# Mariachiar/Spatiotemporal-Deepfake-Detection-for-Live-Video-Calls

Hardware: AMD Instinct MI355X
Metric: clips/sec (32x3x224x224) (higher is better)
Workload: dtype bf16

## Files before the change

spatiotemporal-deepfake-detection-for-live-video-calls_amd/csrc/af_conv.hip:

```cpp
#include "af_common.h"

namespace af {

struct ConvArgs {
    const char* in;
    const char* w;
    const float* scale;
    const float* shift;
    const char* res;
    char* out;
    int T, H, W, Cin, Cout;
    int CinP, CoutP;
    int kt, kh, kw, st, sh, sw, pt, ph, pw;
    int To, Ho, Wo;
    int relu, out_ld;
    int ring;
    int tpool;
    long long M;
    int tiles_n;
    int kpt;
    const char* in2;
    const char* w2;
    int T2, H2, W2, Cin2, Cin2P, st2, sh2, sw2, kpt2;
    int ksplit;
    unsigned div_w_m, div_w_l, div_h_m, div_h_l, div_t_m, div_t_l;
    float* ws;
    long long ws_bytes;
#ifdef AF_STAMPS
    unsigned long long* stamps;
    int dbg;
#endif
};

template <int DT, int BN, int BM, int WN, int WM, int KS, int NSTAGE, int MINW, bool DUAL, bool SPLITK, int BMR>
__device__ __forceinline__ void conv_igemm_tile(const ConvArgs& a, const int bid, const int nb) {
    typedef Elem<DT> E;
    constexpr int EPC = E::EPC;
    constexpr int ES = 16 / EPC;
    constexpr int WTN = BN / WN, WTM = BMR / WM;
    constexpr int TN = WTN / 16, TM = WTM / 16;
    constexpr int NW = WN * WM * KS;
    constexpr int GR = NW * 8;
    constexpr int RW = BN / GR, RX = BM / GR;
    constexpr int PER_WAVE = RW + RX;
    constexpr int STAGE_BYTES = (BN + BM) * 128;
    static_assert(NW == 8 && (KS == 1 || KS == 2) && BN % GR == 0 && BM % GR == 0, "8 waves per workgroup");
    static_assert(BMR <= BM && BMR % (WM * 16) == 0, "real tile rows");
    constexpr bool LEAN = MINW >= 4;
    typedef Mma<DT> MMA;
    static_assert(NSTAGE == 3 || (NSTAGE == 2 && !LEAN && KS == 1), "ring depth of the pipelined loop: 3 or 2 slots");

    extern __shared__ uint4 smem[];
    const unsigned lds0 = (unsigned)(uintptr_t)(__attribute__((address_space(3))) char*)smem;
    AF_STAMP_DECL;
    AF_STAMP(4);

    const int xcd = bid & 7, q = nb >> 3, r = nb & 7;
    const int swz = (xcd < r ? xcd * (q + 1) : r * (q + 1) + (xcd - r) * q) + (bid >> 3);
    const int tile_n = swz % a.tiles_n;
    const int tile_m = swz / a.tiles_n;

    const int tid = threadIdx.x, lane = tid & 63;
    const int wave = __builtin_amdgcn_readfirstlane(tid >> 6);
    const int kgroup = wave / (WN * WM), wsub = wave % (WN * WM);
    const int wn = wsub % WN, wm = wsub / WN;
    const int lrow = tid >> 3;
    const int chunk = (tid & 7) ^ (lrow & 7);

    const int taps = a.kt * a.kh * a.kw;
    const long long m0 = (long long)tile_m * BMR;
    auto row_offsets = [&](long long m, long long& off1, long long& off2, unsigned& mask) {
        const unsigned mq = (unsigned)(a.tpool == 2 ? (m >> 2) : a.tpool ? (m >> 1) : m);
        const unsigned wdiv = (unsigned)(a.tpool == 2 ? (a.Wo >> 1) : a.Wo), hdiv = (unsigned)(a.tpool == 2 ? (a.Ho >> 1) : a.Ho);
        auto fdiv = [](unsigned x, unsigned mm, unsigned l) { const unsigned t = __umulhi(mm, x); return l == 0 ? x : (t + ((x - t) >> 1)) >> (l - 1); };
        const unsigned t1 = fdiv(mq, a.div_w_m, a.div_w_l);
        int wo = (int)(mq - t1 * wdiv);
        const unsigned t2 = fdiv(t1, a.div_h_m, a.div_h_l);
        int ho = (int)(t1 - t2 * hdiv);
        const unsigned tdiv = (unsigned)(a.tpool == 1 ? (a.To >> 1) : a.To);
        const unsigned nq = fdiv(t2, a.div_t_m, a.div_t_l);
        int to = (int)(t2 - nq * tdiv); const long long n = nq;
        if (a.tpool == 1) to = 2 * to + (int)(m & 1);
        if (a.tpool == 2) { ho = 2 * ho + (int)((m >> 1) & 1); wo = 2 * wo + (int)(m & 1); }
        const int ti0 = to * a.st - a.pt, hi0 = ho * a.sh - a.ph, wi0 = wo * a.sw - a.pw;
        off1 = ((((n * a.T + ti0) * a.H + hi0) * a.W + wi0) * a.Cin) * ES;
        off2 = DUAL ? ((((n * a.T2 + to * a.st2) * a.H2 + ho * a.sh2) * a.W2 + wo * a.sw2) * a.Cin2) * ES : 0;
        unsigned mw = 0, mhw = 0, mthw = 0;
        for (int dw = 0; dw < a.kw; ++dw) mw |= ((unsigned)(wi0 + dw) < (unsigned)a.W ? 1u : 0u) << dw;
        for (int dh = 0; dh < a.kh; ++dh) mhw |= ((unsigned)(hi0 + dh) < (unsigned)a.H ? mw : 0u) << (dh * a.kw);
        for (int dt = 0; dt < a.kt; ++dt) mthw |= ((unsigned)(ti0 + dt) < (unsigned)a.T ? mhw : 0u) << (dt * a.kh * a.kw);
        mask = (1u << 31) | mthw;
    };
    const bool flat_rows = !DUAL && taps == 1 && a.tpool == 0 && a.st == 1 && a.sh == 1 && a.sw == 1 && a.pt == 0 && a.ph == 0 && a.pw == 0;
    long long org1, org2; unsigned org_mask;
    if (flat_rows) { org1 = m0 * a.Cin * ES; org2 = 0; }
    else row_offsets(m0, org1, org2, org_mask);
    const i32x4 xdesc = make_desc(a.in + org1);
    const i32x4 x2desc = make_desc((DUAL ? a.in2 : a.in) + org2);
    unsigned xoff[RX], x2off[RX];
    unsigned xmask[RX];
#pragma unroll
    for (int i = 0; i < RX; ++i) {
        const long long m = m0 + lrow + GR * i;
        xmask[i] = 0; xoff[i] = kOutOfRange; x2off[i] = kOutOfRange;
        if (m < a.M && (BMR == BM || lrow + GR * i < BMR)) {
            if (flat_rows) {
                xmask[i] = (1u << 31) | 1u;
                xoff[i] = (unsigned)((lrow + GR * i) * a.Cin * ES) + chunk * 16;
            } else {
                long long o1, o2;
                row_offsets(m, o1, o2, xmask[i]);
                xoff[i] = (unsigned)(o1 - org1) + chunk * 16;
                x2off[i] = (unsigned)(o2 - org2) + chunk * 16;
            }
        }
    }
    const long long Kw = (long long)taps * a.CinP;
    constexpr int BKE = 8 * EPC;
    const bool clast = chunk * EPC < a.Cin - (a.kpt - 1) * BKE;
    const bool clast2 = DUAL && chunk * EPC < a.Cin2 - (a.kpt2 - 1) * BKE;
    const i32x4 wdesc = make_desc(a.w + (long long)tile_n * BN * Kw * ES);
    const i32x4 w2desc = make_desc(a.w2 + (long long)tile_n * BN * a.Cin2P * ES);
    unsigned woff[RW], w2off[RW];
#pragma unroll
    for (int i = 0; i < RW; ++i) {
        woff[i] = (unsigned)(((lrow + GR * i) * Kw + chunk * EPC) * ES);
        w2off[i] = (unsigned)(((long long)(lrow + GR * i) * a.Cin2P + chunk * EPC) * ES);
    }

    int dt = 0, dh = 0, dw = 0, kc = 0, tap = 0;
    auto issue_piece = [&](int st, int g) {
        const unsigned base = lds0 + st * STAGE_BYTES + wave * (8 * 128) + g * (GR * 128);
        if (DUAL && tap >= taps) {
            const int off2 = kc * 128;
            if (g < RW) blds16(w2off[g], w2desc, off2, base);
            else blds16(((xmask[g - RW] >> 31) && (kc + 1 < a.kpt2 || clast2)) ? x2off[g - RW] : kOutOfRange, x2desc, off2, base);
        } else if (g < RW) {
            blds16(woff[g], wdesc, tap * a.CinP * ES + kc * 128, base);
        } else {
            const int xsoff = ((dt * a.H + dh) * a.W + dw) * a.Cin * ES + kc * 128;
            const bool ok = ((xmask[g - RW] >> tap) & 1u) && (kc + 1 < a.kpt || clast);
            blds16(ok ? xoff[g - RW] : kOutOfRange, xdesc, xsoff, base);
        }
    };
    auto advance = [&]() {
        ++kc;
        if (DUAL && tap >= taps) return;
        if (kc == a.kpt) {
            kc = 0; ++tap;
            if (++dw == a.kw) { dw = 0; if (++dh == a.kh) { dh = 0; ++dt; } }
        }
    };
    auto issue_stage = [&](int st) {
#pragma unroll
        for (int g = 0; g < PER_WAVE; ++g) issue_piece(st, g);
        advance();
    };

    f32x4 acc[TN][TM];
#pragma unroll
    for (int i = 0; i < TN; ++i)
#pragma unroll
        for (int j = 0; j < TM; ++j) acc[i][j] = f32x4{0.f, 0.f, 0.f, 0.f};

    const int S_all = taps * a.kpt + (DUAL ? a.kpt2 : 0);
    const int s_lo = SPLITK ? (int)((long long)blockIdx.y * S_all / a.ksplit) : 0;
    const int S = (SPLITK ? (int)((long long)(blockIdx.y + 1) * S_all / a.ksplit) : S_all) - s_lo;
    if (SPLITK) for (int i = 0; i < s_lo; ++i) advance();
    AF_STAMP(0); AF_STAMP(6);
    issue_stage(0);
    if (S > 1 && !(LEAN && a.ring == 2)) issue_stage(1);

    AF_STAMP(1);
    const int frow = lane & 15, fg = lane >> 4;
    constexpr int NKK = 2 / KS;
    const int kk0 = KS == 2 ? kgroup : 0;
    const int wrow = (wn * WTN + frow) * 8, xrow = BN * 8 + (wm * WTM + frow) * 8;
    if constexpr (LEAN || NKK == 1 || TM < 4) {
        auto multiply = [&](int st_) {
            const uint4* ws = smem + st_ * (STAGE_BYTES / 16) + wrow;
            const uint4* xs = smem + st_ * (STAGE_BYTES / 16) + xrow;
#pragma unroll
            for (int q = 0; q < NKK; ++q) {
                const int c = ((kk0 + q) * 4 + fg) ^ (frow & 7);
                uint4 af[TN], bf[TM];
#pragma unroll
                for (int i = 0; i < TN; ++i) af[i] = ws[i * 16 * 8 + c];
#pragma unroll
                for (int j = 0; j < TM; ++j) bf[j] = xs[j * 16 * 8 + c];
#pragma unroll
                for (int i = 0; i < TN; ++i)
#pragma unroll
                    for (int j = 0; j < TM; ++j) MMA::run(af[i], bf[j], acc[i][j]);
            }
        };
        if (LEAN && a.ring == 2) {
            for (int s = 0; s < S; ++s) {
                wait_vmcnt<0>();
                __builtin_amdgcn_s_barrier();
                if (s + 1 < S) issue_stage((s + 1) & 1);
                multiply(s & 1);
            }
        } else {
            int st = 0;
            for (int s = 0; s < S; ++s) {
                if (s + 1 < S) wait_vmcnt<PER_WAVE>(); else wait_vmcnt<0>();
                __builtin_amdgcn_s_barrier();
                if (s + 2 < S) issue_stage(st == 0 ? 2 : st - 1);
                multiply(st);
                st = (st == 2) ? 0 : st + 1;
            }
        }
#ifdef AF_NO_ASM_IGEMM
    } else if constexpr (false) {
#else
    } else if constexpr (DT != AF_F32 && !DUAL && !(LEAN || NKK == 1 || TM < 4)) {
#endif
        constexpr int NTH = TN * TM, NR = TN + TM;
        constexpr int H1 = 3 * NTH / 4;
        static_assert(NR <= H1 && NR + PER_WAVE <= NTH, "reads in front of a LATE wave's barrier; a DMA piece or a read per MFMA");
        u32x4 a0[TN], b0[TM], a1[TN], b1[TM];
        const unsigned wb[2] = {lds0 + (unsigned)((wn * WTN + frow) * 128 + (((0 + fg) ^ (frow & 7)) << 4)),
                                lds0 + (unsigned)((wn * WTN + frow) * 128 + (((4 + fg) ^ (frow & 7)) << 4))};
        const unsigned xb[2] = {lds0 + (unsigned)((BN + wm * WTM + frow) * 128 + (((0 + fg) ^ (frow & 7)) << 4)),
                                lds0 + (unsigned)((BN + wm * WTM + frow) * 128 + (((4 + fg) ^ (frow & 7)) << 4))};
        auto frag_read = [&](u32x4 (&af)[TN], u32x4 (&bf)[TM], unsigned wsb, unsigned xsb, auto idx) {
            constexpr int r = decltype(idx)::value;
            if constexpr (r < TN) af[r] = lds_read16_uncounted<r * (16 * 128)>(wsb);
            else if constexpr (r < NR) bf[r - TN] = lds_read16_uncounted<(r - TN) * (16 * 128)>(xsb);
        };
        auto pin_half = [&](u32x4 (&af)[TN], u32x4 (&bf)[TM]) {
#pragma unroll
            for (int i = 0; i < TN; ++i) pin_frag(af[i]);
#pragma unroll
            for (int j = 0; j < TM; ++j) pin_frag(bf[j]);
        };
        auto mma_group = [&](auto t0c, auto t1c, auto readsc, const u32x4 (&af)[TN], const u32x4 (&bf)[TM], u32x4 (&naf)[TN], u32x4 (&nbf)[TM],
                             unsigned wsb, unsigned xsb) {
            constexpr int T0 = decltype(t0c)::value, T1 = decltype(t1c)::value;
            static_for<T1 - T0>([&](auto tt) {
                constexpr int t = T0 + decltype(tt)::value;
                MmaAsm<DT>::run(af[t / TM], bf[t % TM], acc[t / TM][t % TM]);
                if constexpr (decltype(readsc)::value && t < NR) frag_read(naf, nbf, wsb, xsb, IC<t>{});
            });
        };
        if (NSTAGE == 3 && S > 2) issue_stage(2);
        if (S >= NSTAGE) wait_vmcnt<(NSTAGE - 1) * PER_WAVE>(); else if (S == 2) wait_vmcnt<PER_WAVE>(); else wait_vmcnt<0>();
        __builtin_amdgcn_s_barrier();
        static_for<NR>([&](auto r) { frag_read(a0, b0, wb[0], xb[0], r); });
#pragma unroll
        for (int i = 0; i < TN; ++i)
#pragma unroll
            for (int j = 0; j < TM; ++j) acc_live(acc[i][j]);
        mfma_operands_settled();
        const bool late = wave >= 4;
        int stoff = 0;
        wait_lgkmcnt<0>();
        pin_half(a0, b0);
#pragma nounroll
        for (int s = 0; s < S; ++s) {
            const bool laststep = s + 1 == S;
            const int stnext = stoff == (NSTAGE - 1) * STAGE_BYTES ? 0 : stoff + STAGE_BYTES;
            auto wait_stage = [&]() {
                if (AF_DBG(1)) return;
                if (NSTAGE == 2 || (s == 0 && S <= 2)) wait_vmcnt<0>(); else wait_vmcnt<PER_WAVE>();
            };
            mma_group(IC<0>{}, IC<H1>{}, IC<1>{}, a0, b0, a1, b1, wb[1] + stoff, xb[1] + stoff);
            if (late && !laststep) {
                wait_lgkmcnt<0>();
                wait_stage();
                if (!AF_DBG(2)) __builtin_amdgcn_s_barrier();
            }
            mma_group(IC<H1>{}, IC<NTH>{}, IC<0>{}, a0, b0, a1, b1, 0u, 0u);
            wait_lgkmcnt<0>();
            if (!late && !laststep) {
                wait_stage();
                if (!AF_DBG(2)) __builtin_amdgcn_s_barrier();
            }
            pin_half(a1, b1);
            const bool refill = s + NSTAGE < S && !AF_DBG(4);
            const int wsoff = __builtin_amdgcn_readfirstlane(tap * a.CinP * ES + kc * 128);
            const int xsoff = __builtin_amdgcn_readfirstlane(((dt * a.H + dh) * a.W + dw) * a.Cin * ES + kc * 128);
            i32x4 wd = wdesc, xd = xdesc;
            if (!refill) { wd[2] = 0; xd[2] = 0; }
            const bool lastk = kc + 1 < a.kpt || clast;
            const unsigned tapbit = (unsigned)tap;
            const unsigned dst0 = lds0 + (laststep ? stnext : stoff) + wave * (8 * 128);
            const unsigned wsb0 = wb[0] + stnext, xsb0 = xb[0] + stnext;
            static_for<NTH>([&](auto tc) {
                constexpr int t = tc, slot = group2_slot(t, PER_WAVE, NR);
                MmaAsm<DT>::run(a1[t / TM], b1[t % TM], acc[t / TM][t % TM]);
                if constexpr (slot != kNoSlot && slot < 0) frag_read(a0, b0, wsb0, xsb0, IC<-1 - slot>{});
                else if constexpr (slot != kNoSlot) {
                    constexpr int g = slot;
                    if constexpr (g < RW) blds16_m0(woff[g], wd, wsoff, __builtin_amdgcn_readfirstlane(dst0 + g * (GR * 128)));
                    else {
                        const bool ok = ((xmask[g - RW] >> tapbit) & 1u) && lastk;
                        blds16_m0(ok ? xoff[g - RW] : kOutOfRange, xd, xsoff, __builtin_amdgcn_readfirstlane(dst0 + g * (GR * 128)));
                    }
                }
            });
            if (refill) advance();
            stoff = stnext;
            wait_lgkmcnt<0>();
            pin_half(a0, b0);
        }
        wait_vmcnt<0>();
        mfma_drain();
    } else {
        constexpr int NTH = TN * TM;
        constexpr int MPG = (NTH + PER_WAVE - 1) / PER_WAVE;
        uint4 a0[TN], b0[TM], a1[TN], b1[TM];
        auto read_half = [&](uint4 (&af)[TN], uint4 (&bf)[TM], int st_, int kk) {
            const int c = (kk * 4 + fg) ^ (frow & 7);
            const uint4* ws = smem + st_ * (STAGE_BYTES / 16) + wrow;
            const uint4* xs = smem + st_ * (STAGE_BYTES / 16) + xrow;
#pragma unroll
            for (int i = 0; i < TN; ++i) af[i] = ws[i * 16 * 8 + c];
#pragma unroll
            for (int j = 0; j < TM; ++j) bf[j] = xs[j * 16 * 8 + c];
        };
        int st = 0;
        if (NSTAGE == 2) {
            if (S > 1) wait_vmcnt<PER_WAVE>(); else wait_vmcnt<0>();
            __builtin_amdgcn_s_barrier();
            read_half(a0, b0, 0, 0);
            for (int s = 0; s + 1 < S; ++s) {
                const bool refill = s + 2 < S;
                const int st1 = st ^ 1;
                read_half(a1, b1, st, 1);
                __builtin_amdgcn_sched_barrier(0);
#pragma unroll
                for (int t = 0; t < NTH; ++t) MMA::run(a0[t / TM], b0[t % TM], acc[t / TM][t % TM]);
                __builtin_amdgcn_sched_barrier(0);
                asm volatile("s_waitcnt lgkmcnt(0)" ::: "memory");
                if (!AF_DBG(1)) wait_vmcnt<0>();
                if (!AF_DBG(2)) __builtin_amdgcn_s_barrier();
                read_half(a0, b0, st1, 0);
#pragma unroll
                for (int g = 0; g < PER_WAVE; ++g) {
                    __builtin_amdgcn_sched_barrier(0);
                    if (refill && !AF_DBG(4)) issue_piece(st, g);
                    __builtin_amdgcn_sched_barrier(0);
#pragma unroll
                    for (int t = g * MPG; t < (g + 1) * MPG && t < NTH; ++t) MMA::run(a1[t / TM], b1[t % TM], acc[t / TM][t % TM]);
                }
#pragma unroll
                for (int t = PER_WAVE * MPG; t < NTH; ++t) MMA::run(a1[t / TM], b1[t % TM], acc[t / TM][t % TM]);
                if (refill) advance();
                __builtin_amdgcn_sched_barrier(0);
                st = st1;
            }
        } else {
            wait_vmcnt<0>();
            __builtin_amdgcn_s_barrier();
            read_half(a0, b0, 0, 0);
            for (int s = 0; s + 1 < S; ++s) {
                const bool refill = s + 2 < S;
                const int nst = st == 0 ? 2 : st - 1;
                const int st1 = st == 2 ? 0 : st + 1;
                read_half(a1, b1, st, 1);
#pragma unroll
                for (int g = 0; g < PER_WAVE; ++g) {
                    __builtin_amdgcn_sched_barrier(0);
                    if (refill && !AF_DBG(4)) issue_piece(nst, g);
                    __builtin_amdgcn_sched_barrier(0);
#pragma unroll
                    for (int t = g * MPG; t < (g + 1) * MPG && t < NTH; ++t) MMA::run(a0[t / TM], b0[t % TM], acc[t / TM][t % TM]);
                }
#pragma unroll
                for (int t = PER_WAVE * MPG; t < NTH; ++t) MMA::run(a0[t / TM], b0[t % TM], acc[t / TM][t % TM]);
                if (refill) advance();
                __builtin_amdgcn_sched_barrier(0);
                asm volatile("s_waitcnt lgkmcnt(0)" ::: "memory");
                if (!AF_DBG(1)) { if (refill) wait_vmcnt<PER_WAVE>(); else wait_vmcnt<0>(); }
                if (!AF_DBG(2)) __builtin_amdgcn_s_barrier();
                read_half(a0, b0, st1, 0);
                __builtin_amdgcn_sched_barrier(0);
#pragma unroll
                for (int t = 0; t < NTH; ++t) MMA::run(a1[t / TM], b1[t % TM], acc[t / TM][t % TM]);
                __builtin_amdgcn_sched_barrier(0);
                st = st1;
            }
        }
        read_half(a1, b1, st, 1);
#pragma unroll
        for (int t = 0; t < NTH; ++t) MMA::run(a0[t / TM], b0[t % TM], acc[t / TM][t % TM]);
#pragma unroll
        for (int t = 0; t < NTH; ++t) MMA::run(a1[t / TM], b1[t % TM], acc[t / TM][t % TM]);
    }

    AF_STAMP(2);
    __builtin_amdgcn_s_barrier();
    int patch_off = 0;
    if (KS == 2) {
        f32x4* red = reinterpret_cast<f32x4*>(smem);
        if (kgroup == 1) {
#pragma unroll
            for (int i = 0; i < TN; ++i)
#pragma unroll
                for (int j = 0; j < TM; ++j) red[(wsub * TN * TM + i * TM + j) * 64 + lane] = acc[i][j];
        }
        __builtin_amdgcn_s_barrier();
        if (kgroup == 1) return;
#pragma unroll
        for (int i = 0; i < TN; ++i)
#pragma unroll
            for (int j = 0; j < TM; ++j) acc[i][j] += red[(wsub * TN * TM + i * TM + j) * 64 + lane];
        patch_off = WN * WM * TN * TM * 64 * 4;
    }
    if constexpr (DT != AF_F32 && !SPLITK && KS == 1 && !LEAN) {
        if (a.tpool == 0 && !a.res) {
            typedef typename E::type OT;
            constexpr int PROW16 = WTN + 8;
            OT* patch16 = reinterpret_cast<OT*>(smem) + wsub * (16 * PROW16);
            constexpr int LPR16 = WTN / 8, RPI16 = 64 / LPR16;
            const int rr16 = lane / LPR16, cc16 = (lane % LPR16) * 8;
            const int chb = tile_n * BN + wn * WTN;
            f32x4 sc[TN], sf[TN];
#pragma unroll
            for (int i = 0; i < TN; ++i) {
                sc[i] = *reinterpret_cast<const f32x4*>(a.scale + chb + i * 16 + fg * 4);
                sf[i] = *reinterpret_cast<const f32x4*>(a.shift + chb + i * 16 + fg * 4);
            }
            const float lo = a.relu ? 0.f : -__builtin_inff();
#pragma unroll
            for (int j = 0; j < TM; ++j) {
#pragma unroll
                for (int i = 0; i < TN; ++i) {
                    f32x4 v = acc[i][j] * sc[i] + sf[i];
                    v[0] = max_nan(v[0], lo); v[1] = max_nan(v[1], lo); v[2] = max_nan(v[2], lo); v[3] = max_nan(v[3], lo);
                    Vec4<DT>::store(reinterpret_cast<char*>(patch16 + frow * PROW16 + i * 16 + fg * 4), v);
                }
                __builtin_amdgcn_wave_barrier();
#pragma unroll
                for (int it = 0; it < 16 / RPI16; ++it) {
                    const int row = it * RPI16 + rr16;
                    const long long m = m0 + wm * WTM + j * 16 + row;
                    const u32x4 o = *reinterpret_cast<const u32x4*>(patch16 + row * PROW16 + cc16);
                    if (m < a.M && (BMR == BM || wm * WTM + j * 16 + row < BMR) && chb + cc16 < a.Cout)
                        __builtin_nontemporal_store(o, reinterpret_cast<u32x4*>(a.out + (m * a.out_ld + chb + cc16) * ES));
                }
                __builtin_amdgcn_wave_barrier();
            }
            AF_STAMP(3); AF_STAMP(7);
            AF_STAMP_FLUSH(bid);
            return;
        }
    }
    constexpr int PROW = WTN + 4;
    constexpr int HALVES = TM % 4 == 0 && TM >= 8 ? 4 : TM % 2 == 0 ? 2 : TM;
    constexpr int TMH = TM / HALVES, PROWS = TMH * 16;
    float* patch = reinterpret_cast<float*>(smem) + patch_off + wsub * (PROWS * PROW);
    constexpr int LPR = WTN / EPC;
    constexpr int RPI = 64 / LPR;
    const int rr = lane / LPR, cc = (lane % LPR) * EPC;
    const int ch0 = tile_n * BN + wn * WTN + cc;
#pragma unroll
    for (int hf = 0; hf < HALVES; ++hf) {
#pragma unroll
        for (int i = 0; i < TN; ++i) {
            const int chl = i * 16 + fg * 4;
            const int ch = tile_n * BN + wn * WTN + chl;
            const f32x4 sc = SPLITK ? f32x4{1.f, 1.f, 1.f, 1.f} : *reinterpret_cast<const f32x4*>(a.scale + ch);
            const f32x4 sf = SPLITK ? f32x4{0.f, 0.f, 0.f, 0.f} : *reinterpret_cast<const f32x4*>(a.shift + ch);
#pragma unroll
            for (int j = 0; j < TMH; ++j)
                *reinterpret_cast<f32x4*>(patch + (j * 16 + frow) * PROW + chl) = acc[i][hf * TMH + j] * sc + sf;
        }
        __builtin_amdgcn_wave_barrier();
        if (a.tpool == 2) {
            constexpr int QR = PROWS / 4;
#pragma unroll
            for (int it = 0; it < (QR + RPI - 1) / RPI; ++it) {
                const bool live = it * RPI + rr < QR;
                const int prow = live ? it * RPI + rr : 0;
                const long long m = m0 + wm * WTM + hf * PROWS + 4 * prow;
                float v[EPC];
#pragma unroll
                for (int p4 = 0; p4 < 4; ++p4)
#pragma unroll
                    for (int e = 0; e < EPC; e += 4) {
                        const f32x4 t = *reinterpret_cast<const f32x4*>(patch + (4 * prow + p4) * PROW + cc + e);
#pragma unroll
                        for (int q = 0; q < 4; ++q) {
                            const float x = a.relu ? relu_f(t[q]) : t[q];
                            v[e + q] = p4 == 0 ? x : max_nan(v[e + q], x);
                        }
                    }
                if (live && m < a.M && ch0 < a.Cout) {
                    uint4 o;
                    typename E::type* oe = reinterpret_cast<typename E::type*>(&o);
#pragma unroll
                    for (int e = 0; e < EPC; ++e) oe[e] = E::from_f32(v[e]);
                    __builtin_nontemporal_store(__builtin_bit_cast(u32x4, o), reinterpret_cast<u32x4*>(a.out + ((m >> 2) * a.out_ld + ch0) * ES));
                }
            }
        } else if (a.tpool) {
#pragma unroll
            for (int it = 0; it < PROWS / (2 * RPI); ++it) {
                const int prow = it * RPI + rr;
                const long long m = m0 + wm * WTM + hf * PROWS + 2 * prow;
                float v[2][EPC];
#pragma unroll
                for (int p2 = 0; p2 < 2; ++p2)
#pragma unroll
                    for (int e = 0; e < EPC; e += 4) {
                        const f32x4 t = *reinterpret_cast<const f32x4*>(patch + (2 * prow + p2) * PROW + cc + e);
                        v[p2][e] = t[0]; v[p2][e + 1] = t[1]; v[p2][e + 2] = t[2]; v[p2][e + 3] = t[3];
                    }
                if (m < a.M && ch0 < a.Cout) {
                    if (a.res) {
                        const long long mq = m >> 1, hw = (long long)a.Ho * a.Wo;
                        const long long pix = mq % hw, nj = mq / hw;
                        const long long lin0 = (nj * 2) * hw + pix;
#pragma unroll
                        for (int p2 = 0; p2 < 2; ++p2) {
                            const uint4 rraw = __builtin_bit_cast(uint4, __builtin_nontemporal_load(reinterpret_cast<const u32x4*>(a.res + ((lin0 + p2 * hw) * a.Cout + ch0) * ES)));
                            const typename E::type* re = reinterpret_cast<const typename E::type*>(&rraw);
#pragma unroll
                            for (int e = 0; e < EPC; ++e) v[p2][e] += E::to_f32(re[e]);
                        }
                    }
                    uint4 o;
                    typename E::type* oe = reinterpret_cast<typename E::type*>(&o);
#pragma unroll
                    for (int e = 0; e < EPC; ++e) {
                        float x0 = v[0][e], x1 = v[1][e];
                        if (a.relu) { x0 = relu_f(x0); x1 = relu_f(x1); }
                        oe[e] = E::from_f32(max_nan(x0, x1));
                    }
                    __builtin_nontemporal_store(__builtin_bit_cast(u32x4, o), reinterpret_cast<u32x4*>(a.out + ((m >> 1) * a.out_ld + ch0) * ES));
                }
            }
        } else {
#pragma unroll
            for (int it = 0; it < PROWS / RPI; ++it) {
                const int row = it * RPI + rr;
                const long long m = m0 + wm * WTM + hf * PROWS + row;
                float v[EPC];
#pragma unroll
                for (int e = 0; e < EPC; e += 4) {
                    const f32x4 t = *reinterpret_cast<const f32x4*>(patch + row * PROW + cc + e);
                    v[e] = t[0]; v[e + 1] = t[1]; v[e + 2] = t[2]; v[e + 3] = t[3];
                }
                if (SPLITK) {
                    if (m < a.M && ch0 < a.Cout) {
                        float* wp = a.ws + ((long long)blockIdx.y * a.M + m) * a.Cout + ch0;
#pragma unroll
                        for (int e = 0; e < EPC; e += 4)
                            *reinterpret_cast<f32x4*>(wp + e) = f32x4{v[e], v[e + 1], v[e + 2], v[e + 3]};
                    }
                } else if (m < a.M && ch0 < a.Cout) {
                    if (a.res) {
                        const uint4 rraw = __builtin_bit_cast(uint4, __builtin_nontemporal_load(reinterpret_cast<const u32x4*>(a.res + (m * a.Cout + ch0) * ES)));
                        const typename E::type* re = reinterpret_cast<const typename E::type*>(&rraw);
#pragma unroll
                        for (int e = 0; e < EPC; ++e) v[e] += E::to_f32(re[e]);
                    }
                    if (a.relu) {
#pragma unroll
                        for (int e = 0; e < EPC; ++e) v[e] = relu_f(v[e]);
                    }
                    uint4 o;
                    typename E::type* oe = reinterpret_cast<typename E::type*>(&o);
#pragma unroll
                    for (int e = 0; e < EPC; ++e) oe[e] = E::from_f32(v[e]);
                    __builtin_nontemporal_store(__builtin_bit_cast(u32x4, o), reinterpret_cast<u32x4*>(a.out + (m * a.out_ld + ch0) * ES));
                }
            }
        }
        __builtin_amdgcn_wave_barrier();
    }
    AF_STAMP(3); AF_STAMP(7);
    AF_STAMP_FLUSH(bid);
}

template <int DT, int BN, int BM, int WN, int WM, int KS, int NSTAGE, int MINW, bool DUAL, bool SPLITK, int BMR>
__global__ __launch_bounds__(WN * WM * KS * 64, MINW) void conv_igemm_kernel(const ConvArgs a) {
    conv_igemm_tile<DT, BN, BM, WN, WM, KS, NSTAGE, MINW, DUAL, SPLITK, BMR>(a, blockIdx.x, gridDim.x);
}

static long long igemm_tiles(long long M, int bmr, int tiles_n) { return (M + bmr - 1) / bmr * tiles_n; }

template <int DT, int BN, int BM, int WN, int WM, int KS, int MINW, bool DUAL, int NSTAGE = 3, bool SPLITK = false, int BMR = BM>
static int launch(const ConvArgs& a, hipStream_t stream) {
    const long long blocks = igemm_tiles(a.M, BMR, a.tiles_n);
    if (blocks <= 0 || blocks > 0x7fffffffLL) return set_error(AF_ERR_ARG, "conv: grid of %lld workgroups", blocks);
    constexpr int TMv = BMR / WM / 16;
    constexpr int red_bytes = KS == 2 ? WN * WM * (BN / WN / 16) * TMv * 64 * 16 : 0;
    constexpr int patch_bytes = red_bytes + WN * WM * ((TMv % 4 == 0 && TMv >= 8 ? TMv / 4 : TMv % 2 == 0 ? TMv / 2 : 1) * 16) * (BN / WN + 4) * 4;
    const int S = a.kt * a.kh * a.kw * a.kpt + a.kpt2;
    const int slots = (MINW >= 4 && a.ring == 2) ? 2 : NSTAGE;
    const int ring_bytes = (S < slots ? S : slots) * (BN + BM) * 128;
    const int lds = ring_bytes > patch_bytes ? ring_bytes : patch_bytes;
    AF_SET_MAX_LDS((&conv_igemm_kernel<DT, BN, BM, WN, WM, KS, NSTAGE, MINW, DUAL, SPLITK, BMR>),
                   NSTAGE * (BN + BM) * 128 > patch_bytes ? NSTAGE * (BN + BM) * 128 : patch_bytes, "conv");
    hipLaunchKernelGGL((conv_igemm_kernel<DT, BN, BM, WN, WM, KS, NSTAGE, MINW, DUAL, SPLITK, BMR>), dim3((unsigned)blocks, SPLITK ? a.ksplit : 1), dim3(WN * WM * KS * 64), lds, stream, a);
    AF_CHECK_LAUNCH("conv_igemm_kernel");
    return AF_OK;
}

enum { VAR_128x256 = 0, VAR_64x256 = 1, VAR_128x128 = 2, VAR_64x128 = 3, VAR_C133 = 4, VAR_128x128_R2 = 5, VAR_256x256 = 6,
       VAR_128x512 = 7, VAR_C311 = 8, VAR_SMALL = 9, VAR_C111 = 10, VAR_C133G = 11, VAR_256x224 = 12, VAR_C311G = 13, VAR_COUNT = 14 };

struct Variant { const char* name; int bn, bm, wn, wm, ks, minw, nstage, bmr, ring; bool dual; };
constexpr Variant variant_info(int v) {
    switch (v) {
        case VAR_128x256: return {"conv_igemm<BN=128,BM=256>", 128, 256, 2, 4, 1, 2, 3, 256, 3, true};
        case VAR_64x256: return {"conv_igemm<BN=64,BM=256>", 64, 256, 1, 8, 1, 2, 3, 256, 3, true};
        case VAR_128x128: return {"conv_igemm<BN=128,BM=128>", 128, 128, 2, 4, 1, 6, 3, 128, 3, true};
        case VAR_128x128_R2: return {"conv_igemm<BN=128,BM=128>", 128, 128, 2, 4, 1, 6, 3, 128, 2, true};
        case VAR_64x128: return {"conv_igemm<BN=64,BM=128>", 64, 128, 1, 8, 1, 4, 3, 128, 3, true};
        case VAR_256x256: return {"conv_igemm<BN=256,BM=256>", 256, 256, 2, 4, 1, 2, 2, 256, 3, true};
        case VAR_256x224: return {"conv_igemm<BN=256,BM=224>", 256, 256, 4, 2, 1, 2, 2, 224, 3, true};
        case VAR_128x512: return {"conv_igemm<BN=128,BM=512>", 128, 512, 2, 4, 1, 2, 2, 512, 3, false};
        case VAR_C133: return {"conv133_c64<weights in registers>"};
        case VAR_C311: return {"conv311_c64<time-tiled, taps share one LDS image>"};
        case VAR_SMALL: return {"conv_small<direct-gather MFMA, narrow layers>"};
        case VAR_C111: return {"conv111<persistent stream, weights in registers>"};
        case VAR_C133G: return {"conv133g<frame-resident halo patch, 9 taps share it>"};
        case VAR_C311G: return {"conv311g<clip-resident (T + 2) x P patch, 3 taps share it>"};
        default: return {"?"};
    }
}
static int variant_bm(int v) { return variant_info(v).bmr; }
static int variant_bn(int v) { return variant_info(v).bn; }

static int pick_variant(int cout, int cin, int taps, int dtype, long long M, int cin2 = 0, int pooled = 0) {
    if (const char* fv = getenv("AF_FORCE_VAR")) {
        const int v = atoi(fv);
        const int bn = variant_bn(v);
        const bool generic = bn != 0;
        if (generic && cout % bn == 0 && !(pooled && v == VAR_256x224)) return v;
    }
    const int ksteps = (taps * cin + cin2) / (dtype == AF_F32 ? 32 : 64);
    const bool wide = cout % 128 == 0, short_k = ksteps <= 3;
    if (cout % 256 == 0 && ksteps >= (pooled == 2 ? 4 : cin2 ? 6 : 9)) {
        const int mode224 = env_int("AF_IGEMM_224", 1);
        const long long tm = (M + 255) / 256, big = tm * (cout / 256), v0 = tm * (cout / 128);
        const long long b224 = (M + 223) / 224 * (cout / 256);
        const double c256 = (double)((big + 255) / 256), c224 = 0.89 * (double)((b224 + 255) / 256);
        const bool take224 = pooled == 0 && mode224 != 0 && (mode224 == 2 || (M % 49 == 0 && c224 < c256 - 0.02));
        if (big >= 128 && (take224 ? c224 : c256) < 0.615 * (double)((v0 + 255) / 256) + 0.05) return take224 ? VAR_256x224 : VAR_256x256;
    }
    if (cout == 128 && !cin2 && taps >= 9) {
        const long long big = (M + 511) / 512, v0 = (M + 255) / 256;
        if (big >= 128 && (double)((big + 255) / 256) < 0.615 * (double)((v0 + 255) / 256) + 0.05) return VAR_128x512;
    }
    if ((M + 255) / 256 * (cout / (wide ? 128 : 64)) < 64) return VAR_64x128;
    if (wide && !short_k && ksteps <= 8 && (cout >= 512 || cout == 128)) return VAR_128x128_R2;
    return wide ? (short_k ? VAR_128x128 : VAR_128x256) : (short_k ? VAR_64x128 : VAR_64x256);
}

template <int DT>
__global__ void splitk_finish_kernel(const float* ws, int ksplit, long long M, int Cout, const float* scale, const float* shift,
                                     const char* res, int relu, char* out, int out_ld) {
    constexpr int ES = 16 / Elem<DT>::EPC;
    const long long i = (long long)blockIdx.x * blockDim.x + threadIdx.x, per_row = Cout / 4;
    if (i >= M * per_row) return;
    const long long m = i / per_row;
    const int c = (int)(i % per_row) * 4;
    f32x4 v = f32x4{0.f, 0.f, 0.f, 0.f};
    for (int y = 0; y < ksplit; ++y) v += *reinterpret_cast<const f32x4*>(ws + ((long long)y * M + m) * Cout + c);
    v = v * *reinterpret_cast<const f32x4*>(scale + c) + *reinterpret_cast<const f32x4*>(shift + c);
    if (res) v += Vec4<DT>::load(res + (m * Cout + c) * ES);
    if (relu) { v[0] = relu_f(v[0]); v[1] = relu_f(v[1]); v[2] = relu_f(v[2]); v[3] = relu_f(v[3]); }
    Vec4<DT>::store(out + (m * out_ld + c) * ES, v);
}

static int plan_ksplit(int v, long long M, int coutp, int cout, int s_all, int tpool, bool dual) {
    const long long blocks = (M + variant_bm(v) - 1) / variant_bm(v) * (coutp / variant_bn(v));
    if (tpool || dual || blocks >= 128 || s_all < 16 || cout % 4 != 0) return 1;
    int ks = (int)(256 / blocks);
    if (ks > 8) ks = 8;
    if (ks > s_all / 8) ks = s_all / 8;
    return ks >= 2 ? ks : 1;
}

struct ConvPad { int coutp, cinp, cin2p, kpt, kpt2, taps, ksteps; long long M; };
static ConvPad conv_pad(const af_conv_desc* d, const af_conv_desc* d2) {
    const int bk = d->dtype == AF_F32 ? 32 : 64;
    ConvPad p;
    p.coutp = (d->cout + 63) / 64 * 64;
    p.kpt = (d->cin + bk - 1) / bk; p.cinp = p.kpt * bk;
    p.kpt2 = d2 ? (d2->cin + bk - 1) / bk : 0; p.cin2p = p.kpt2 * bk;
    p.taps = d->kt * d->kh * d->kw; p.ksteps = p.taps * p.kpt + p.kpt2;
    p.M = (long long)d->n * d->to * d->ho * d->wo;
    return p;
}
static int pick_variant(const af_conv_desc* d, const ConvPad& p) { return pick_variant(p.coutp, p.cinp, p.taps, d->dtype, p.M, p.cin2p, d->tpool); }

static int conv_path(const af_conv_desc* d, const af_conv_desc* d2, const void* residual, int out_ld, const ConvPad& p) {
    if (conv_small_applies(d, d2, residual, out_ld)) return VAR_SMALL;
    if (!d2 && conv133_applies(d, residual, out_ld)) return VAR_C133;
    if (!d2 && conv133g_applies(d, residual, out_ld)) return VAR_C133G;
    if (!d2 && conv311g_applies(d, residual, out_ld)) return VAR_C311G;
    if (!d2 && conv311_applies(d, residual, out_ld)) return VAR_C311;
    if (conv111_applies(d, d2, residual, out_ld)) return VAR_C111;
    return pick_variant(d, p);
}

template <int DT, bool DUAL, bool SPLITK, int V = 0>
static int launch_variant(int v, const ConvArgs& a, hipStream_t stream) {
    constexpr Variant t = variant_info(V < VAR_COUNT ? V : VAR_64x128);
    if constexpr (V < VAR_COUNT && (t.bn == 0 || (DUAL && !t.dual))) return launch_variant<DT, DUAL, SPLITK, V + 1>(v, a, stream);
    else {
        if constexpr (V < VAR_COUNT) if (v != V) return launch_variant<DT, DUAL, SPLITK, V + 1>(v, a, stream);
        return launch<DT, t.bn, t.bm, t.wn, t.wm, t.ks, t.minw, DUAL, t.nstage, SPLITK, t.bmr>(a, stream);
    }
}

template <int DT>
static int dispatch(ConvArgs& a, const ConvPad& p, int v, hipStream_t stream) {
    a.kpt = p.kpt; a.CinP = p.cinp; a.kpt2 = p.kpt2; a.Cin2P = p.cin2p; a.CoutP = p.coutp;
    a.tiles_n = a.CoutP / variant_bn(v);
    a.ring = variant_info(v).ring;
    a.ksplit = plan_ksplit(v, a.M, a.CoutP, a.Cout, p.ksteps, a.tpool, a.in2 != nullptr);
    if (a.ksplit > 1 && (!a.ws || a.ws_bytes < (long long)a.ksplit * a.M * a.Cout * (long long)sizeof(float))) a.ksplit = 1;
    const int rc = a.in2 ? launch_variant<DT, true, false>(v, a, stream)
                   : a.ksplit > 1 ? launch_variant<DT, false, true>(v, a, stream) : launch_variant<DT, false, false>(v, a, stream);
    if (rc != AF_OK || a.ksplit == 1) return rc;
    const long long quads = a.M * (a.Cout / 4);
    hipLaunchKernelGGL((splitk_finish_kernel<DT>), dim3((unsigned)((quads + 255) / 256)), dim3(256), 0, stream, a.ws, a.ksplit, a.M, a.Cout,
                       a.scale, a.shift, a.res, a.relu, a.out, a.out_ld);
    AF_CHECK_LAUNCH("splitk_finish_kernel");
    return AF_OK;
}

}

extern "C" int af_conv_variant(const af_conv_desc* d, const af_conv_desc* d2) {
    AF_REQUIRE(d && d->cout > 0 && d->cin > 0 && af::dtype_ok(d->dtype), "conv_variant: bad descriptor");
    return af::conv_path(d, d2, nullptr, 0, af::conv_pad(d, d2));
}

extern "C" int af_conv_work_units(const af_conv_desc* d, const af_conv_desc* d2, int64_t* units, int* workgroups) {
    using namespace af;
    AF_REQUIRE(d && units && workgroups && d->cout > 0 && d->cin > 0 && dtype_ok(d->dtype), "conv_work_units: bad argument");
    AF_REQUIRE(d->n > 0 && d->to > 0 && d->ho > 0 && d->wo > 0, "conv_work_units: bad dims");
    const ConvPad p = conv_pad(d, d2);
    const int v = conv_path(d, d2, nullptr, 0, p);
    long long u = 0;
    int g = 0;
    switch (v) {
        case VAR_C133: conv133_work(d, &u, &g); break;
        case VAR_C133G: conv133g_work(d, &u, &g); break;
        case VAR_C311G: conv311g_work(d, &u, &g); break;
        case VAR_C311: conv311_work(d, &u, &g); break;
        case VAR_C111: conv111_work(d, d2, &u, &g); break;
        case VAR_SMALL: return set_error(AF_ERR_ARG, "conv_work_units: the narrow-layer path is not cut into units");
// ... 159 lines not shown
```

Baseline: 3425.

## Prefetch residual and BN params during main loop, defer activation offset setup

Stages the per-channel BN scale/shift into LDS at kernel start so the epilogue reads them from shared memory instead of global. Issues weight loads for stage 0 before computing activation row offsets, which hides the address math behind the first loads. For eligible tile configs it also issues residual-tile loads during the last K-step and double-buffers them across epilogue halves. The cost is more LDS, more registers and extra template instantiations, which may reduce occupancy.

```diff
diff --git a/spatiotemporal-deepfake-detection-for-live-video-calls_amd/csrc/af_conv.hip b/spatiotemporal-deepfake-detection-for-live-video-calls_amd/csrc/af_conv.hip
--- a/spatiotemporal-deepfake-detection-for-live-video-calls_amd/csrc/af_conv.hip
+++ b/spatiotemporal-deepfake-detection-for-live-video-calls_amd/csrc/af_conv.hip
@@ -26,13 +26,25 @@
     unsigned div_w_m, div_w_l, div_h_m, div_h_l, div_t_m, div_t_l;
     float* ws;
     long long ws_bytes;
+    int res_pre;
+    int bn_off;
 #ifdef AF_STAMPS
     unsigned long long* stamps;
     int dbg;
 #endif
 };
 
-template <int DT, int BN, int BM, int WN, int WM, int KS, int NSTAGE, int MINW, bool DUAL, bool SPLITK, int BMR>
+constexpr int kBnLdsBytes = 2 * 1024;
+constexpr bool bn_in_lds(int bn, int bm, int nstage, bool splitk) { return !splitk && nstage * (bn + bm) * 128 + kBnLdsBytes <= 160 * 1024; }
+
+constexpr int kResPreRows = 2;
+constexpr bool res_prefetched(int dt, int bn, int wn, int wm, int bmr, int minw, bool dual, bool splitk) {
+    const int epc = dt == AF_F32 ? 4 : 8, wtn = bn / wn, tm = bmr / wm / 16;
+    const int halves = tm % 4 == 0 && tm >= 8 ? 4 : tm % 2 == 0 ? 2 : tm, prows = tm / halves * 16, rpi = 64 / (wtn / epc);
+    return !dual && !splitk && (minw >= 4 || tm < 4) && prows % (2 * rpi) == 0 && prows / rpi <= kResPreRows;
+}
+
+template <int DT, int BN, int BM, int WN, int WM, int KS, int NSTAGE, int MINW, bool DUAL, bool SPLITK, int BMR, bool RESP>
 __device__ __forceinline__ void conv_igemm_tile(const ConvArgs& a, const int bid, const int nb) {
     typedef Elem<DT> E;
     constexpr int EPC = E::EPC;
@@ -47,6 +59,14 @@
     static_assert(NW == 8 && (KS == 1 || KS == 2) && BN % GR == 0 && BM % GR == 0, "8 waves per workgroup");
     static_assert(BMR <= BM && BMR % (WM * 16) == 0, "real tile rows");
     constexpr bool LEAN = MINW >= 4;
+    constexpr bool BN_LDS = bn_in_lds(BN, BM, NSTAGE, SPLITK);
+    constexpr int PROW = WTN + 4;
+    constexpr int HALVES = TM % 4 == 0 && TM >= 8 ? 4 : TM % 2 == 0 ? 2 : TM;
+    constexpr int TMH = TM / HALVES, PROWS = TMH * 16;
+    constexpr int LPR = WTN / EPC;
+    constexpr int RPI = 64 / LPR;
+    constexpr int NRH = PROWS / RPI;
+    constexpr bool RES_PRE = RESP && KS == 1 && res_prefetched(DT, BN, WN, WM, BMR, MINW, DUAL, SPLITK);
     typedef Mma<DT> MMA;
     static_assert(NSTAGE == 3 || (NSTAGE == 2 && !LEAN && KS == 1), "ring depth of the pipelined loop: 3 or 2 slots");
 
@@ -91,30 +111,6 @@
         for (int dt = 0; dt < a.kt; ++dt) mthw |= ((unsigned)(ti0 + dt) < (unsigned)a.T ? mhw : 0u) << (dt * a.kh * a.kw);
         mask = (1u << 31) | mthw;
     };
-    const bool flat_rows = !DUAL && taps == 1 && a.tpool == 0 && a.st == 1 && a.sh == 1 && a.sw == 1 && a.pt == 0 && a.ph == 0 && a.pw == 0;
-    long long org1, org2; unsigned org_mask;
-    if (flat_rows) { org1 = m0 * a.Cin * ES; org2 = 0; }
-    else row_offsets(m0, org1, org2, org_mask);
-    const i32x4 xdesc = make_desc(a.in + org1);
-    const i32x4 x2desc = make_desc((DUAL ? a.in2 : a.in) + org2);
-    unsigned xoff[RX], x2off[RX];
-    unsigned xmask[RX];
-#pragma unroll
-    for (int i = 0; i < RX; ++i) {
-        const long long m = m0 + lrow + GR * i;
-        xmask[i] = 0; xoff[i] = kOutOfRange; x2off[i] = kOutOfRange;
-        if (m < a.M && (BMR == BM || lrow + GR * i < BMR)) {
-            if (flat_rows) {
-                xmask[i] = (1u << 31) | 1u;
-                xoff[i] = (unsigned)((lrow + GR * i) * a.Cin * ES) + chunk * 16;
-            } else {
-                long long o1, o2;
-                row_offsets(m, o1, o2, xmask[i]);
-                xoff[i] = (unsigned)(o1 - org1) + chunk * 16;
-                x2off[i] = (unsigned)(o2 - org2) + chunk * 16;
-            }
-        }
-    }
     const long long Kw = (long long)taps * a.CinP;
     constexpr int BKE = 8 * EPC;
     const bool clast = chunk * EPC < a.Cin - (a.kpt - 1) * BKE;
@@ -127,6 +123,10 @@
         woff[i] = (unsigned)(((lrow + GR * i) * Kw + chunk * EPC) * ES);
         w2off[i] = (unsigned)(((long long)(lrow + GR * i) * a.Cin2P + chunk * EPC) * ES);
     }
+
+    i32x4 xdesc, x2desc;
+    unsigned xoff[RX], x2off[RX];
+    unsigned xmask[RX];
 
     int dt = 0, dh = 0, dw = 0, kc = 0, tap = 0;
     auto issue_piece = [&](int st, int g) {
@@ -168,9 +168,66 @@
     const int S = (SPLITK ? (int)((long long)(blockIdx.y + 1) * S_all / a.ksplit) : S_all) - s_lo;
     if (SPLITK) for (int i = 0; i < s_lo; ++i) advance();
     AF_STAMP(0); AF_STAMP(6);
-    issue_stage(0);
+    if constexpr (BN_LDS) {
+        if (wave < 2)
+            blds16(lane * 4 < BN ? lane * 16u : kOutOfRange, make_desc(reinterpret_cast<const char*>(wave == 0 ? a.scale : a.shift)),
+                   __builtin_amdgcn_readfirstlane(tile_n * BN * 4), __builtin_amdgcn_readfirstlane(lds0 + a.bn_off + wave * (kBnLdsBytes / 2)));
+    }
+#pragma unroll
+    for (int g = 0; g < RW; ++g) issue_piece(0, g);
+    __builtin_amdgcn_sched_barrier(0);
+    const bool flat_rows = !DUAL && taps == 1 && a.tpool == 0 && a.st == 1 && a.sh == 1 && a.sw == 1 && a.pt == 0 && a.ph == 0 && a.pw == 0;
+    long long org1, org2; unsigned org_mask;
+    if (flat_rows) { org1 = m0 * a.Cin * ES; org2 = 0; }
+    else row_offsets(m0, org1, org2, org_mask);
+    xdesc = make_desc(a.in + org1);
+    x2desc = make_desc((DUAL ? a.in2 : a.in) + org2);
+#pragma unroll
+    for (int i = 0; i < RX; ++i) {
+        const long long m = m0 + lrow + GR * i;
+        xmask[i] = 0; xoff[i] = kOutOfRange; x2off[i] = kOutOfRange;
+        if (m < a.M && (BMR == BM || lrow + GR * i < BMR)) {
+            if (flat_rows) {
+                xmask[i] = (1u << 31) | 1u;
+                xoff[i] = (unsigned)((lrow + GR * i) * a.Cin * ES) + chunk * 16;
+            } else {
+                long long o1, o2;
+                row_offsets(m, o1, o2, xmask[i]);
+                xoff[i] = (unsigned)(o1 - org1) + chunk * 16;
+                x2off[i] = (unsigned)(o2 - org2) + chunk * 16;
+            }
+        }
+    }
+#pragma unroll
+    for (int g = RW; g < PER_WAVE; ++g) issue_piece(0, g);
+    advance();
     if (S > 1 && !(LEAN && a.ring == 2)) issue_stage(1);
 
+    u32x4 rpre[RES_PRE ? NRH : 1];
+    auto request_slice0 = [&]() {
+        int lane_p = lane;
+        asm volatile("" : "+v"(lane_p));
+        const int rr_p = lane_p / LPR, ch0_p = tile_n * BN + wn * WTN + (lane_p % LPR) * EPC;
+        const bool want = a.res_pre && ch0_p < a.Cout;
+        const long long hw = (long long)a.Ho * a.Wo;
+        const unsigned mq0 = (unsigned)(m0 >> 1), uhw = (unsigned)hw;
+        const long long lin_org = a.tpool ? (long long)(mq0 / uhw) * 2 * hw + mq0 % uhw : m0;
+        const i32x4 rdesc = make_desc((a.res_pre ? a.res : a.in) + lin_org * a.Cout * ES);
+#pragma unroll
+        for (int it = 0; it < (RES_PRE ? NRH : 0); ++it) {
+            long long m, lin;
+            if (a.tpool) {
+                m = m0 + wm * WTM + 2 * ((it >> 1) * RPI + rr_p);
+                const unsigned mq = (unsigned)(m >> 1);
+                lin = (long long)(mq / uhw) * 2 * hw + mq % uhw + (it & 1) * hw;
+            } else {
+                m = m0 + wm * WTM + it * RPI + rr_p;
+                lin = m;
+            }
+            const unsigned voff = (unsigned)(((lin - lin_org) * a.Cout + ch0_p) * ES);
+            rpre[it] = bload16_nt_uncounted(want && m < a.M ? voff : kOutOfRange, rdesc, 0);
+        }
+    };
     AF_STAMP(1);
     const int frow = lane & 15, fg = lane >> 4;
     constexpr int NKK = 2 / KS;
@@ -195,20 +252,34 @@
             }
         };
         if (LEAN && a.ring == 2) {
-            for (int s = 0; s < S; ++s) {
+            for (int s = 0; s < S - (RES_PRE ? 1 : 0); ++s) {
                 wait_vmcnt<0>();
                 __builtin_amdgcn_s_barrier();
                 if (s + 1 < S) issue_stage((s + 1) & 1);
                 multiply(s & 1);
             }
+            if constexpr (RES_PRE) {
+                request_slice0();
+                wait_vmcnt<RES_PRE ? NRH : 0>();
+                __builtin_amdgcn_s_barrier();
+                multiply((S - 1) & 1);
+                wait_vmcnt<0>();
+            }
         } else {
             int st = 0;
-            for (int s = 0; s < S; ++s) {
+            for (int s = 0; s < S - (RES_PRE ? 1 : 0); ++s) {
                 if (s + 1 < S) wait_vmcnt<PER_WAVE>(); else wait_vmcnt<0>();
                 __builtin_amdgcn_s_barrier();
                 if (s + 2 < S) issue_stage(st == 0 ? 2 : st - 1);
                 multiply(st);
                 st = (st == 2) ? 0 : st + 1;
+            }
+            if constexpr (RES_PRE) {
+                request_slice0();
+                wait_vmcnt<RES_PRE ? NRH : 0>();
+                __builtin_amdgcn_s_barrier();
+                multiply(st);
+                wait_vmcnt<0>();
             }
         }
 #ifdef AF_NO_ASM_IGEMM
@@ -393,6 +464,8 @@
     AF_STAMP(2);
     __builtin_amdgcn_s_barrier();
     int patch_off = 0;
+    const float* bn_sc = BN_LDS ? reinterpret_cast<const float*>(reinterpret_cast<const char*>(smem) + a.bn_off) : a.scale + tile_n * BN;
+    const float* bn_sf = BN_LDS ? bn_sc + kBnLdsBytes / 8 : a.shift + tile_n * BN;
     if (KS == 2) {
         f32x4* red = reinterpret_cast<f32x4*>(smem);
         if (kgroup == 1) {
@@ -420,8 +493,8 @@
             f32x4 sc[TN], sf[TN];
 #pragma unroll
             for (int i = 0; i < TN; ++i) {
-                sc[i] = *reinterpret_cast<const f32x4*>(a.scale + chb + i * 16 + fg * 4);
-                sf[i] = *reinterpret_cast<const f32x4*>(a.shift + chb + i * 16 + fg * 4);
+                sc[i] = *reinterpret_cast<const f32x4*>(bn_sc + wn * WTN + i * 16 + fg * 4);
+                sf[i] = *reinterpret_cast<const f32x4*>(bn_sf + wn * WTN + i * 16 + fg * 4);
             }
             const float lo = a.relu ? 0.f : -__builtin_inff();
 #pragma unroll
@@ -448,22 +521,40 @@
             return;
         }
     }
-    constexpr int PROW = WTN + 4;
-    constexpr int HALVES = TM % 4 == 0 && TM >= 8 ? 4 : TM % 2 == 0 ? 2 : TM;
-    constexpr int TMH = TM / HALVES, PROWS = TMH * 16;
     float* patch = reinterpret_cast<float*>(smem) + patch_off + wsub * (PROWS * PROW);
-    constexpr int LPR = WTN / EPC;
-    constexpr int RPI = 64 / LPR;
     const int rr = lane / LPR, cc = (lane % LPR) * EPC;
     const int ch0 = tile_n * BN + wn * WTN + cc;
+    u32x4 rcur[RES_PRE ? NRH : 1];
+    if constexpr (RES_PRE) {
+#pragma unroll
+        for (int k = 0; k < NRH; ++k) { asm volatile("" : "+v"(rpre[k])); rcur[k] = rpre[k]; }
+    }
+    auto request_slice = [&](int hf, u32x4 (&r)[RES_PRE ? NRH : 1]) {
+        const long long hw = (long long)a.Ho * a.Wo;
+#pragma unroll
+        for (int k = 0; k < (RES_PRE ? NRH : 0); ++k) {
+            long long m, lin;
+            if (a.tpool) {
+                m = m0 + wm * WTM + hf * PROWS + 2 * ((k >> 1) * RPI + rr);
+                const long long mq = m >> 1;
+                lin = (mq / hw) * 2 * hw + mq % hw + (k & 1) * hw;
+            } else {
+                m = m0 + wm * WTM + hf * PROWS + k * RPI + rr;
+                lin = m;
+            }
+            r[k] = u32x4{0u, 0u, 0u, 0u};
+            if (m < a.M && ch0 < a.Cout) r[k] = __builtin_nontemporal_load(reinterpret_cast<const u32x4*>(a.res + (lin * a.Cout + ch0) * ES));
+        }
+    };
 #pragma unroll
     for (int hf = 0; hf < HALVES; ++hf) {
+        u32x4 rnxt[RES_PRE ? NRH : 1];
+        if (RES_PRE && a.res_pre && hf + 1 < HALVES) request_slice(hf + 1, rnxt);
 #pragma unroll
         for (int i = 0; i < TN; ++i) {
             const int chl = i * 16 + fg * 4;
-            const int ch = tile_n * BN + wn * WTN + chl;
-            const f32x4 sc = SPLITK ? f32x4{1.f, 1.f, 1.f, 1.f} : *reinterpret_cast<const f32x4*>(a.scale + ch);
-            const f32x4 sf = SPLITK ? f32x4{0.f, 0.f, 0.f, 0.f} : *reinterpret_cast<const f32x4*>(a.shift + ch);
+            const f32x4 sc = SPLITK ? f32x4{1.f, 1.f, 1.f, 1.f} : *reinterpret_cast<const f32x4*>(bn_sc + wn * WTN + chl);
+            const f32x4 sf = SPLITK ? f32x4{0.f, 0.f, 0.f, 0.f} : *reinterpret_cast<const f32x4*>(bn_sf + wn * WTN + chl);
 #pragma unroll
             for (int j = 0; j < TMH; ++j)
                 *reinterpret_cast<f32x4*>(patch + (j * 16 + frow) * PROW + chl) = acc[i][hf * TMH + j] * sc + sf;
@@ -516,7 +607,9 @@
                         const long long lin0 = (nj * 2) * hw + pix;
 #pragma unroll
                         for (int p2 = 0; p2 < 2; ++p2) {
-                            const uint4 rraw = __builtin_bit_cast(uint4, __builtin_nontemporal_load(reinterpret_cast<const u32x4*>(a.res + ((lin0 + p2 * hw) * a.Cout + ch0) * ES)));
+                            uint4 rraw;
+                            if (RES_PRE && a.res_pre) rraw = __builtin_bit_cast(uint4, rcur[RES_PRE ? 2 * it + p2 : 0]);
+                            else rraw = __builtin_bit_cast(uint4, __builtin_nontemporal_load(reinterpret_cast<const u32x4*>(a.res + ((lin0 + p2 * hw) * a.Cout + ch0) * ES)));
                             const typename E::type* re = reinterpret_cast<const typename E::type*>(&rraw);
 #pragma unroll
                             for (int e = 0; e < EPC; ++e) v[p2][e] += E::to_f32(re[e]);
@@ -553,7 +646,9 @@
                     }
                 } else if (m < a.M && ch0 < a.Cout) {
                     if (a.res) {
-                        const uint4 rraw = __builtin_bit_cast(uint4, __builtin_nontemporal_load(reinterpret_cast<const u32x4*>(a.res + (m * a.Cout + ch0) * ES)));
+                        uint4 rraw;
+                        if (RES_PRE && a.res_pre) rraw = __builtin_bit_cast(uint4, rcur[RES_PRE ? it : 0]);
+                        else rraw = __builtin_bit_cast(uint4, __builtin_nontemporal_load(reinterpret_cast<const u32x4*>(a.res + (m * a.Cout + ch0) * ES)));
                         const typename E::type* re = reinterpret_cast<const typename E::type*>(&rraw);
 #pragma unroll
                         for (int e = 0; e < EPC; ++e) v[e] += E::to_f32(re[e]);
@@ -571,14 +666,18 @@
             }
         }
         __builtin_amdgcn_wave_barrier();
+        if constexpr (RES_PRE && HALVES > 1) {
+#pragma unroll
+            for (int k = 0; k < NRH; ++k) rcur[k] = rnxt[k];
+        }
     }
     AF_STAMP(3); AF_STAMP(7);
     AF_STAMP_FLUSH(bid);
 }
 
-template <int DT, int BN, int BM, int WN, int WM, int KS, int NSTAGE, int MINW, bool DUAL, bool SPLITK, int BMR>
+template <int DT, int BN, int BM, int WN, int WM, int KS, int NSTAGE, int MINW, bool DUAL, bool SPLITK, int BMR, bool RESP = false>
 __global__ __launch_bounds__(WN * WM * KS * 64, MINW) void conv_igemm_kernel(const ConvArgs a) {
-    conv_igemm_tile<DT, BN, BM, WN, WM, KS, NSTAGE, MINW, DUAL, SPLITK, BMR>(a, blockIdx.x, gridDim.x);
+    conv_igemm_tile<DT, BN, BM, WN, WM, KS, NSTAGE, MINW, DUAL, SPLITK, BMR, RESP>(a, blockIdx.x, gridDim.x);
 }
 
 static long long igemm_tiles(long long M, int bmr, int tiles_n) { return (M + bmr - 1) / bmr * tiles_n; }
@@ -593,10 +692,26 @@
     const int S = a.kt * a.kh * a.kw * a.kpt + a.kpt2;
     const int slots = (MINW >= 4 && a.ring == 2) ? 2 : NSTAGE;
     const int ring_bytes = (S < slots ? S : slots) * (BN + BM) * 128;
-    const int lds = ring_bytes > patch_bytes ? ring_bytes : patch_bytes;
-    AF_SET_MAX_LDS((&conv_igemm_kernel<DT, BN, BM, WN, WM, KS, NSTAGE, MINW, DUAL, SPLITK, BMR>),
-                   NSTAGE * (BN + BM) * 128 > patch_bytes ? NSTAGE * (BN + BM) * 128 : patch_bytes, "conv");
-    hipLaunchKernelGGL((conv_igemm_kernel<DT, BN, BM, WN, WM, KS, NSTAGE, MINW, DUAL, SPLITK, BMR>), dim3((unsigned)blocks, SPLITK ? a.ksplit : 1), dim3(WN * WM * KS * 64), lds, stream, a);
+    constexpr bool BN_LDS = bn_in_lds(BN, BM, NSTAGE, SPLITK);
+    constexpr int full_ring = NSTAGE * (BN + BM) * 128;
+    const int ring_extent = (MINW >= 4 || !BN_LDS) ? ring_bytes : full_ring;
+    ConvArgs b = a;
+    constexpr bool RES_PRE = KS == 1 && res_prefetched(DT, BN, WN, WM, BMR, MINW, DUAL, SPLITK);
+    b.res_pre = RES_PRE && a.res && a.tpool != 2 &&
+                (BMR + 2LL * a.Ho * a.Wo + 2) * a.Cout * (DT == AF_F32 ? 4 : 2) < (1LL << 31);
+    b.bn_off = ring_extent > patch_bytes ? ring_extent : patch_bytes;
+    const int lds = b.bn_off + (BN_LDS ? kBnLdsBytes : 0);
+    constexpr int max_lds = (full_ring > patch_bytes ? full_ring : patch_bytes) + (BN_LDS ? kBnLdsBytes : 0);
+    if constexpr (RES_PRE) {
+        if (b.res_pre) {
+            AF_SET_MAX_LDS((&conv_igemm_kernel<DT, BN, BM, WN, WM, KS, NSTAGE, MINW, DUAL, SPLITK, BMR, true>), max_lds, "conv");
+            hipLaunchKernelGGL((conv_igemm_kernel<DT, BN, BM, WN, WM, KS, NSTAGE, MINW, DUAL, SPLITK, BMR, true>), dim3((unsigned)blocks, 1), dim3(WN * WM * KS * 64), lds, stream, b);
+            AF_CHECK_LAUNCH("conv_igemm_kernel");
+            return AF_OK;
+        }
+    }
+    AF_SET_MAX_LDS((&conv_igemm_kernel<DT, BN, BM, WN, WM, KS, NSTAGE, MINW, DUAL, SPLITK, BMR>), max_lds, "conv");
+    hipLaunchKernelGGL((conv_igemm_kernel<DT, BN, BM, WN, WM, KS, NSTAGE, MINW, DUAL, SPLITK, BMR>), dim3((unsigned)blocks, SPLITK ? a.ksplit : 1), dim3(WN * WM * KS * 64), lds, stream, b);
     AF_CHECK_LAUNCH("conv_igemm_kernel");
     return AF_OK;
 }
```

After: 3430, median of 6. No clear change (+0.2%).
